# MoZhou1995/DeepPDE_ActorCritic

Measured on AMD Instinct MI355X. Metric: SDE trajectory-steps/sec (batch×horizon) at d=20; value-fn rel-L2 vs analytic, higher is better.
Workload: dtype f32

## Files before the change

### deeppde_actorcritic_amd/csrc/dpac_device.h

```cpp
#pragma once

#include <hip/hip_runtime.h>
#include <rocrand/rocrand_kernel.h>
#include <stdint.h>

#include "dpac.h"
#include "dpac_mfma.h"

namespace dpac {

__host__ __device__ constexpr int pow2_at_least(int v) {
  int p = 1;
  while (p < v) p *= 2;
  return p;
}
#ifndef DPAC_LANE_CAP
#define DPAC_LANE_CAP 16
#endif
#ifndef DPAC_LANE_COMPS
#define DPAC_LANE_COMPS 2
#endif
__host__ __device__ constexpr int lanes_for_dim(int D) {
  return pow2_at_least((D + DPAC_LANE_COMPS - 1) / DPAC_LANE_COMPS) < DPAC_LANE_CAP
             ? pow2_at_least((D + DPAC_LANE_COMPS - 1) / DPAC_LANE_COMPS)
             : DPAC_LANE_CAP;
}
__host__ __device__ constexpr int comps_per_lane(int D) {
  return (D + lanes_for_dim(D) - 1) / lanes_for_dim(D);
}
__host__ __device__ constexpr int eqn_lanes(int eqn, int D) {
  return eqn == DPAC_EQN_VDP ? 1 : lanes_for_dim(D);
}

template <int D, int P>
struct Own {
  static constexpr int M = (D + P - 1) / P;
  static constexpr bool kFull = (D % M) == 0;
  int p;
  __device__ __forceinline__ explicit Own(int p_) : p(p_) {}
  __device__ __forceinline__ int j(int m) const { return p * M + m; }
  __device__ __forceinline__ bool valid(int m) const { return p * M + m < D; }
  __device__ __forceinline__ bool active() const { return p * M < D; }
  template <typename T>
  __device__ __forceinline__ void mask(T (&v)[M]) const {
#pragma unroll
    for (int m = 0; m < M; ++m) v[m] = valid(m) ? v[m] : T(0);
  }
  template <typename T>
  __device__ __forceinline__ void load_masked(const T* __restrict__ row, T (&v)[M]) const {
#pragma unroll
    for (int m = 0; m < M; ++m) v[m] = valid(m) ? row[p * M + m] : T(0);
  }
  template <typename T>
  __device__ __forceinline__ void store(T* __restrict__ row, const T (&v)[M]) const {
#pragma unroll
    for (int m = 0; m < M; ++m)
      if (valid(m)) row[p * M + m] = v[m];
  }
};

struct TdRows {
  const void *x, *u, *dw;
  int64_t ldx;
  int ldu, p;
  double sa, sb;
  void* gdot;
  const void* g_gdot;
};

constexpr uint32_t kOOB = 0x80000000u;
constexpr int kRsrcFlags = 0x00020000;

__device__ __forceinline__ __amdgpu_buffer_rsrc_t make_rsrc(const void* base, uint32_t bytes) {
  return __builtin_amdgcn_make_buffer_rsrc(const_cast<void*>(base), 0, (int)bytes, kRsrcFlags);
}

constexpr float kX3Range = 32768.f;
__device__ __forceinline__ bool x3_bad4(float a, float b, float c, float d) {
  return !(fabsf(a) < kX3Range) | !(fabsf(b) < kX3Range) | !(fabsf(c) < kX3Range) | !(fabsf(d) < kX3Range);
}
__device__ __forceinline__ bool x3_bad(float a) { return !(fabsf(a) < kX3Range); }
__device__ __forceinline__ void x3_flag(uint32_t* st) {
  if (st) __hip_atomic_fetch_or(st, 1u, __ATOMIC_RELAXED, __HIP_MEMORY_SCOPE_AGENT);
}
__device__ __forceinline__ bool x3_status_set(const uint32_t* st) {
  return st && __hip_atomic_load(const_cast<uint32_t*>(st), __ATOMIC_RELAXED, __HIP_MEMORY_SCOPE_AGENT) != 0u;
}
// ... 101 lines not shown
      for (int m = 0; m < M; ++m) {
        uint32_t w[sizeof(T) / 4];
        buf_load_dwords<sizeof(T) / 4, AUX>(r, off[m], w, soff);
        __builtin_memcpy(&v[m], &w[0], sizeof(T));
      }
    }
  }
  template <int AUX = 0>
  __device__ __forceinline__ void store(__amdgpu_buffer_rsrc_t r, const T (&v)[M], uint32_t soff = 0) const {
    if constexpr (kVec) {
      uint32_t w[K];
      __builtin_memcpy(&w[0], &v[0], sizeof(w));
      buf_store_dwords<K, AUX>(r, off[0], w, soff);
    } else {
#pragma unroll
      for (int m = 0; m < M; ++m) {
        uint32_t w[sizeof(T) / 4];
        __builtin_memcpy(&w[0], &v[m], sizeof(T));
        buf_store_dwords<sizeof(T) / 4, AUX>(r, off[m], w, soff);
      }
    }
  }
};

template <int CTRL>
__device__ __forceinline__ int dpp_i32(int v) {
  return __builtin_amdgcn_mov_dpp(v, CTRL, 0xF, 0xF, true);
}
template <int CTRL>
__device__ __forceinline__ float dpp(float v) {
  return __builtin_bit_cast(float, dpp_i32<CTRL>(__builtin_bit_cast(int, v)));
}
template <int CTRL>
__device__ __forceinline__ double dpp(double v) {
  const long long b = __builtin_bit_cast(long long, v);
  const int lo = dpp_i32<CTRL>(static_cast<int>(b));
  const int hi = dpp_i32<CTRL>(static_cast<int>(b >> 32));
  return __builtin_bit_cast(double,
                            (static_cast<long long>(hi) << 32) | static_cast<unsigned int>(lo));
}
enum : int {
  kDppXor1 = 0xB1,
  kDppXor2 = 0x4E,
  kDppHalfMirror = 0x141,
  kDppMirror = 0x140,
};

__device__ __forceinline__ float row_pair_sum(float v) {
  const unsigned u = __builtin_bit_cast(unsigned, v);
  const auto sw = __builtin_amdgcn_permlane16_swap(u, u, false, false);
  return __builtin_bit_cast(float, (unsigned)sw[0]) + __builtin_bit_cast(float, (unsigned)sw[1]);
}
__device__ __forceinline__ double row_pair_sum(double v) {
  const unsigned long long u = __builtin_bit_cast(unsigned long long, v);
  const unsigned lo = (unsigned)u, hi = (unsigned)(u >> 32);
  const auto sl = __builtin_amdgcn_permlane16_swap(lo, lo, false, false);
  const auto sh = __builtin_amdgcn_permlane16_swap(hi, hi, false, false);
  const double a = __builtin_bit_cast(double, ((unsigned long long)(unsigned)sh[0] << 32) | (unsigned)sl[0]);
  const double b = __builtin_bit_cast(double, ((unsigned long long)(unsigned)sh[1] << 32) | (unsigned)sl[1]);
  return a + b;
}

template <int P, typename T>
__device__ __forceinline__ T group_shift_in(T keep, T v, bool group_start) {
  if constexpr (P == 1) {
    return v;
  } else {
    constexpr int kRowShr1 = 0x111;
    T sh;
    if constexpr (sizeof(T) == 4) {
      sh = __builtin_bit_cast(T, __builtin_amdgcn_update_dpp(__builtin_bit_cast(int, v),
                                                            __builtin_bit_cast(int, keep),
                                                            kRowShr1, 0xF, 0xF, false));
    } else {
      const long long vb = __builtin_bit_cast(long long, v), kb = __builtin_bit_cast(long long, keep);
      const int lo = __builtin_amdgcn_update_dpp((int)vb, (int)kb, kRowShr1, 0xF, 0xF, false);
      const int hi = __builtin_amdgcn_update_dpp((int)(vb >> 32), (int)(kb >> 32), kRowShr1, 0xF, 0xF,
                                                 false);
      sh = __builtin_bit_cast(T, ((long long)hi << 32) | (unsigned int)lo);
    }
    if constexpr (P < 16) sh = group_start ? v : sh;
    return sh;
  }
}

template <int P>
struct Lanes {
  static_assert(P == 1 || P == 2 || P == 4 || P == 8 || P == 16 || P == 32, "bad group size");
  template <typename T>
  __device__ __forceinline__ static T sum(T v) {
    if constexpr (P >= 2) v = v + dpp<kDppXor1>(v);
    if constexpr (P >= 4) v = v + dpp<kDppXor2>(v);
    if constexpr (P >= 8) v = v + dpp<kDppHalfMirror>(v);
    if constexpr (P >= 16) v = v + dpp<kDppMirror>(v);
    if constexpr (P >= 32) v = row_pair_sum(v);
    return v;
  }
};

enum : uint64_t { kTagDw = 0, kTagDir = 1, kTagRadius = 2, kTagBdry = 3 };

__device__ __forceinline__ uint4 philox_block(uint64_t seed, uint64_t subseq, uint64_t block) {
  rocrand_state_philox4x32_10 st;
  rocrand_init(seed, subseq, block * 4ull, &st);
  return rocrand4(&st);
}

__device__ __forceinline__ void box_muller_hw(unsigned int x, unsigned int y, float& a, float& b) {
  const float u = ROCRAND_2POW32_INV + (x * ROCRAND_2POW32_INV);
  const float v = ROCRAND_2POW32_INV_2PI + (y * ROCRAND_2POW32_INV_2PI);
  const float s = __builtin_amdgcn_sqrtf(-2.0f * __logf(u));
  float sn, cs;
  __sincosf(v, &sn, &cs);
  a = sn * s;
  b = cs * s;
}

template <typename T>
struct Rng;
template <>
struct Rng<float> {
  static constexpr int kNormalPerBlock = 4;
  __device__ __forceinline__ static void normals(uint4 v, float (&o)[4]) {
    box_muller_hw(v.x, v.y, o[0], o[1]);
    box_muller_hw(v.z, v.w, o[2], o[3]);
  }
};
template <>
struct Rng<double> {
  static constexpr int kNormalPerBlock = 2;
  __device__ __forceinline__ static void normals(uint4 v, double (&o)[2]) {
    const double2 n = rocrand_device::detail::normal_distribution_double2(v);
    o[0] = n.x;
    o[1] = n.y;
  }
};

template <typename T>
__device__ __forceinline__ T bounded_value(unsigned int w) {
  const unsigned int k = static_cast<unsigned int>((static_cast<unsigned long long>(w) * 6ull) >> 32);
  const T s3 = static_cast<T>(1.7320508075688772);
  return k == 0u ? -s3 : (k == 5u ? s3 : static_cast<T>(0));
}

template <typename T>
__host__ __device__ constexpr int dw_per_block(int sample_type) {
  return sample_type == DPAC_SAMPLE_BOUNDED ? 4 : (sizeof(T) == 4 ? 4 : 2);
}

template <typename T>
__host__ __device__ constexpr int dw_steps_per_block(int M, int sample_type) {
  return 2 * M <= dw_per_block<T>(sample_type) ? 2 : 1;
}

template <typename T>
__device__ __forceinline__ void dw_block_values(uint64_t seed, uint64_t traj, uint64_t block,
                                                int sample_type, T (&v)[4]) {
  const uint4 w = philox_block(seed, traj, (kTagDw << 48) | block);
  if (sample_type == DPAC_SAMPLE_BOUNDED) {
    v[0] = bounded_value<T>(w.x); v[1] = bounded_value<T>(w.y);
    v[2] = bounded_value<T>(w.z); v[3] = bounded_value<T>(w.w);
  } else {
    T n[Rng<T>::kNormalPerBlock];
    Rng<T>::normals(w, n);
#pragma unroll
    for (int e = 0; e < Rng<T>::kNormalPerBlock; ++e) v[e] = n[e];
// ... 285 lines not shown
  __device__ __forceinline__ void Lop(const T* v, T* o) const {
#pragma unroll
    for (int i = 0; i < C; ++i) o[i] = two_a * v[i] - eps * (v[nxt(i)] + v[prv(i)]);
  }
  __device__ __forceinline__ void u_true(const T (&x)[M], T, T (&u)[MC]) const {
    T dv2[C];
    Lop(x + C, dv2);
#pragma unroll
    for (int i = 0; i < C; ++i) u[i] = -dv2[i] / 2 / q;
  }
  __device__ __forceinline__ void drift(const T (&x)[M], const T (&u)[MC], T, T (&f)[M]) const {
#pragma unroll
    for (int i = 0; i < C; ++i) {
      const T x1 = x[i], x2 = x[C + i];
      f[i] = x2;
      f[C + i] = (1 - x1 * x1) * x2 - x1 + u[i];
    }
  }
  __device__ __forceinline__ void sigma(const T (&x)[M], const T (&u)[MC], T (&s)[M]) const {
#pragma unroll
    for (int m = 0; m < M; ++m) s[m] = sqrt2;
  }
  static void sigma_form(const dpac_eqn_params&, double& sa, double& sb) { sa = 1.4142135623730951; sb = 0.0; }
  __device__ __forceinline__ T w_part(const T (&x)[M], const T (&u)[MC]) const {
    T dv1[C], dv2[C];
    Lop(x, dv1);
    Lop(x + C, dv2);
    T acc = 0;
#pragma unroll
    for (int i = 0; i < C; ++i) {
      const T x1 = x[i], x2 = x[C + i];
      const T px1 = x[nxt(i)], px2 = x[C + nxt(i)];
      const T temp = geps * (x1 * px1 + x2 * px2) + (dv2[i] * dv2[i]) / 4 / q - x2 * dv1[i] -
                     ((1 - x1 * x1) * x2 - x1) * dv2[i];
      acc += temp + q * (u[i] * u[i]) + ga * (x1 * x1 + x2 * x2);
    }
    return acc;
  }
  __device__ __forceinline__ T w_finish(T s) const { return s - two_ad; }
  __device__ __forceinline__ T V_true(const T (&x)[M], T S, T r) const {
    T cross = 0;
#pragma unroll
    for (int i = 0; i < C; ++i) cross += x[i] * x[nxt(i)] + x[C + i] * x[C + nxt(i)];
    return a * S - eps * cross;
  }
  __device__ __forceinline__ T Z(const T (&x)[M], T S, T r) const { return V_true(x, S, r); }
  __device__ __forceinline__ void V_grad(const T (&x)[M], T S, T r, T (&g)[M]) const {
    Lop(x, g);
    Lop(x + C, g + C);
  }
  __device__ __forceinline__ void drift_vjp(const T (&x)[M], const T (&u)[MC], T r, const T (&a)[M],
                            T (&gx)[M], T (&gu)[MC]) const {
#pragma unroll
    for (int i = 0; i < C; ++i) {
      const T x1 = x[i], x2 = x[C + i], a1 = a[i], a2v = a[C + i];
      gx[i] += a2v * (-2 * x1 * x2 - 1);
      gx[C + i] += a1 + a2v * (1 - x1 * x1);
      gu[i] += a2v;
    }
  }
  __device__ __forceinline__ void sigma_vjp(const T (&x)[M], const T (&u)[MC], const T (&a)[M], T (&gx)[M],
                            T (&gu)[MC]) const {}
  __device__ __forceinline__ void w_vjp(const T (&x)[M], const T (&u)[MC], T gw, T (&gx)[M], T (&gu)[MC]) const {
    T dv1[C], dv2[C], g[C], Ldv2[C], Lg[C];
    Lop(x, dv1);
    Lop(x + C, dv2);
#pragma unroll
    for (int i = 0; i < C; ++i) g[i] = (1 - x[i] * x[i]) * x[C + i] - x[i];
    Lop(dv2, Ldv2);
    Lop(g, Lg);
#pragma unroll
    for (int i = 0; i < C; ++i) {
      const T x1 = x[i], x2 = x[C + i];
      const T s1 = x[nxt(i)] + x[prv(i)], s2 = x[C + nxt(i)] + x[C + prv(i)];
      const T d1 = geps * s1 + 2 * x1 * x2 * dv2[i] + two_ga * x1;
      const T d2 = geps * s2 + Ldv2[i] * inv2q - dv1[i] - (1 - x1 * x1) * dv2[i] - Lg[i] + two_ga * x2;
      gx[i] += gw * d1;
      gx[C + i] += gw * d2;
      gu[i] += gw * (two_q * u[i]);
    }
  }
};

}
```

### deeppde_actorcritic_amd/csrc/dpac_eqn_lqr.hip

```cpp
#include "dpac_kernels.h"

namespace dpac {
template <typename T, int D>
using EqLQRFor = EqLQR<T, D, eqn_lanes(DPAC_EQN_LQR, D)>;
namespace {
const Registrar<EqLQRFor, std::conditional_t<DPAC_TU_DOUBLE, double, float>, DPAC_DIMS> reg(DPAC_EQN_LQR);
}
}

#if DPAC_NN_TRACE && DPAC_TU_TRACE
extern "C" int dpac_debug_trace(void* host, int64_t bytes) {
  const int64_t n = bytes < (int64_t)sizeof(dpac::g_nn_trace) ? bytes : (int64_t)sizeof(dpac::g_nn_trace);
  return (int)hipMemcpyFromSymbol(host, HIP_SYMBOL(dpac::g_nn_trace), (size_t)n, 0, hipMemcpyDeviceToHost);
}
#endif
```

### deeppde_actorcritic_amd/csrc/dpac_kernels.h

```cpp
#pragma once

#include <cmath>
#include <type_traits>
#include <utility>

#include "dpac_device.h"

namespace dpac {

enum Op : int {
  OP_ROLLOUT = 0,
  OP_FLAG_INIT,
  OP_STEP_FWD,
  OP_STEP_BWD,
  OP_TD_FWD,
  OP_TD_BWD,
  OP_EVAL,
  OP_ROLLOUT_NN,
  OP_ROLLOUT_NN_BWD,
};

inline int nn_mask_tile_bytes(int n_hidden) { return 13 * 64 * n_hidden; }

struct OpArgs {
  int op;
  dpac_eqn_params eq;
  int scheme, dtype, td_type, cost_order, sample_type, what;
  int64_t B, traj_offset;
  int N;
  double T;
  uint64_t seed;
  const void *x0, *dw, *x, *u, *dt_in, *coef_in, *G, *disc_in, *y_in;
  const int32_t* flag_in;
  const void *g_x_out, *g_disc_out, *g_y_out;
  void *x_out, *dt, *coef, *u_out, *y, *disc, *disc_out, *y_out;
  int32_t* flag_out;
  void *g_x, *g_u, *g_disc, *g_G, *out;
  dpac_mlp mlp;
  void *save_z, *save_disc;
  int32_t* save_flag;
  uint8_t* save_mask;
  int32_t* mask_written;
  const uint8_t* mask_in;
  const void* mlp_wt[DPAC_MLP_MAX_HIDDEN + 1];
  hipStream_t stream;
};

inline HostConsts host_consts(const OpArgs& a) {
  HostConsts h;
  const double d = a.eq.dim;
  h.gamma = a.eq.gamma;
  h.R = a.eq.R;
  h.sigma_up = a.eq.sigma_up;
  h.dt0 = a.T / a.N;
  h.sqrt_dt0 = std::sqrt(h.dt0);
  h.dt_min = h.dt0 * 1e-4;
  h.den = 3 * a.eq.dim * (a.eq.sigma_up * a.eq.sigma_up);
  h.c_layer = a.eq.sigma_up * std::sqrt(3 * d * h.dt0);
  h.R2 = a.eq.R * a.eq.R;
  return h;
}

template <typename T>
struct DevConsts {
  T gamma, R, dt0, sqrt_dt0, dt_min, inv_den, two_inv_den, c_layer, R2, neg_gamma;
  static DevConsts make(const HostConsts& h) {
    DevConsts c;
    c.gamma = (T)h.gamma; c.R = (T)h.R; c.dt0 = (T)h.dt0; c.sqrt_dt0 = (T)h.sqrt_dt0;
    c.dt_min = (T)h.dt_min; c.inv_den = (T)(1.0 / h.den); c.two_inv_den = (T)(2.0 / h.den);
    c.c_layer = (T)h.c_layer; c.R2 = (T)h.R2; c.neg_gamma = (T)(-h.gamma);
    return c;
  }
};

#ifndef DPAC_RING_VGPRS
#define DPAC_RING_VGPRS 32
#endif
#ifndef DPAC_ROLLOUT_KB_CAP
#define DPAC_ROLLOUT_KB_CAP 8
#endif
#ifndef DPAC_ROLLOUT_DW_AUX
#define DPAC_ROLLOUT_DW_AUX 0
#endif
#ifndef DPAC_ROLLOUT_X_AUX
#define DPAC_ROLLOUT_X_AUX 2
// ... 240 lines not shown
#pragma unroll
            for (int m = 0; m < M; ++m) {
              fr.dw[m] = v[m];
              pend[m] = v[M + m];
            }
          } else {
#pragma unroll
            for (int m = 0; m < M; ++m) fr.dw[m] = pend[m];
          }
          return;
        }
      }
      draw_owned<T, E, D>(a.seed, gtraj, t, lc.p, a.sample_type, fr.dw);
    } else if constexpr (DPAC_ABLATE == 2 || DPAC_ABLATE == 5) {
#pragma unroll
      for (int m = 0; m < M; ++m) fr.dw[m] = T(((t * 7 + m + lc.p) & 3) - 1.5) * T(0.5);
    } else {
      sx.template load<DPAC_ROLLOUT_DW_AUX>(rs_dw, fr.dw, (uint32_t)t * slab);
    }
  };
  auto body = [&](int t, DwFrame<T, M>& fr, auto phase) {
    T dwv[M];
#pragma unroll
    for (int m = 0; m < M; ++m) dwv[m] = fr.dw[m];
    if constexpr (PHILOX) own.mask(dwv);
    T u[MC];
    eq.u_true(x, r, u);
    TR tr;
    tr.run(eq, c, x, u, dwv, fl, r);
    const T cf = tr.coef ? T(1) : T(0);
    if constexpr (COST) {
      const T w = eq.w_finish(Lanes<P>::sum(eq.w_part(x, u)));
      y += cost_increment(a.cost_order, w, cf, tr.dt, disc);
      disc = disc * disc_factor(tr.dt, cf, c);
    }
#pragma unroll
    for (int m = 0; m < M; ++m) x[m] = tr.coef ? tr.xt[m] : x[m];
    if constexpr (TR::kRadius) r = tr.coef ? tr.rt : r;
    fl = tr.next;
    if constexpr (DPAC_ABLATE == 1 || DPAC_ABLATE == 5) {
      if (t + 1 == a.N) sx.store(rs_x, x, (uint32_t)(t + 1) * slab);
      return;
    }
    if constexpr (DPAC_ABLATE != 4) sx.template store<DPAC_ROLLOUT_X_AUX>(rs_x, x, (uint32_t)(t + 1) * slab);
    if constexpr (WANT_U) su.store(rs_u, u, (uint32_t)t * slab_u);
    if constexpr (DPAC_ABLATE != 3) {
      constexpr int PH = decltype(phase)::value;
      keep = group_shift_in<P>(keep, tr.coef ? tr.dt : -tr.dt, lc.p == 0);
      if constexpr (PH >= 0) {
        if constexpr (PH % F == F - 1) flush(t, F);
      } else if ((t & (F - 1)) == F - 1) {
        flush(t, F);
      }
    }
  };
  pipelined<KB, DwFrame<T, M>>(0, a.N, load, body);
  if constexpr (DPAC_ABLATE != 3 && DPAC_ABLATE != 1 && DPAC_ABLATE != 5) {
    const int rem = a.N & (F - 1);
    if (rem) flush(a.N - 1, rem);
  }
  if constexpr (COST) {
    if (lc.live && lc.p == 0) {
      a.y[lc.b] = y;
      a.disc[lc.b] = disc;
    }
  }
}

#ifndef DPAC_ST_CHUNKS
#define DPAC_ST_CHUNKS 4
#endif
#ifndef DPAC_ST_TIGHT
#define DPAC_ST_TIGHT 0
#endif
#ifndef DPAC_ST_TIGHT_CHUNKS
#define DPAC_ST_TIGHT_CHUNKS 3
#endif
#ifndef DPAC_ST_PD
#define DPAC_ST_PD 1
#endif
constexpr int kStCW = 4;
constexpr int kStCH = 16;
constexpr int kStPD = DPAC_ST_PD;
static_assert(kStPD >= 1 && kStPD <= kStCH, "prefetch distance within a chunk");
template <typename T, int D, int P>
struct StagedPlan {
  static constexpr int TPW = kStCW * (64 / P);
  static constexpr int SLOT = TPW * D * (int)sizeof(T);
  static constexpr int PIECES = (SLOT + 1023) / 1024;
  static constexpr int kLdsCap = 128 * 1024;
  static constexpr int SLOT_1K = (SLOT + 16 + 1023) / 1024 * 1024;
  static constexpr int SLOT_16 = (SLOT + 16 + 15) / 16 * 16;
  static constexpr bool kWide = !DPAC_ST_TIGHT && DPAC_ST_CHUNKS * kStCH * SLOT_1K <= kLdsCap;
  static constexpr int CHUNKS = kWide ? DPAC_ST_CHUNKS : DPAC_ST_TIGHT_CHUNKS;
  static constexpr int SLOT_LDS = kWide ? SLOT_1K : SLOT_16;
  static constexpr int PADOFF = SLOT_LDS - 16;
  static constexpr int RS = CHUNKS * kStCH;
  static_assert(P < 4 || (SLOT % 16 == 0 && (PIECES - 1) * 1024 + 16 <= SLOT), "DMA pieces stay inside the slot");
  static constexpr bool kOk = P >= 4 && RS * SLOT_LDS <= kLdsCap && kStCH * PIECES <= 62;
};

template <class Fn, int... S>
__device__ __forceinline__ void unroll_phases(Fn& fn, std::integer_sequence<int, S...>) {
  (fn(Phase<S>{}), ...);
}

__device__ __forceinline__ int lds_load_relaxed(const int* p) {
  return __hip_atomic_load(p, __ATOMIC_RELAXED, __HIP_MEMORY_SCOPE_WORKGROUP);
}
__device__ __forceinline__ void lds_store_relaxed(int* p, int v) {
  __hip_atomic_store(p, v, __ATOMIC_RELAXED, __HIP_MEMORY_SCOPE_WORKGROUP);
}

template <int GEN>
constexpr int st_waves() { return kStCW + (GEN > 0 ? GEN : 1); }
#ifndef DPAC_ST_GEN
#define DPAC_ST_GEN 12
#endif
constexpr int kStGen = DPAC_ST_GEN;

template <typename T, class E, int D, int SCHEME, int OUT, int KB, int GEN = 0>
__global__ __launch_bounds__(64 * st_waves<GEN>()) void k_rollout_staged(const E eq, const DevConsts<T> c,
                                                                          const RolloutArgs<T> a) {
  constexpr int P = E::kP, M = E::M, MC = E::MC;
  using PL = StagedPlan<T, D, P>;
  constexpr int TPW = PL::TPW, RS = PL::RS, PIECES = PL::PIECES, SLOT_LDS = PL::SLOT_LDS;
  constexpr bool COST = (OUT & kOutCost) != 0, WANT_U = (OUT & kOutU) != 0;
  constexpr int F = P < kStCH ? P : kStCH;
  constexpr int NREADY = GEN > 0 ? GEN : 1;
  static_assert(kStCH % F == 0 && (F & (F - 1)) == 0, "flush phase fixed per unrolled body");
  static_assert(GEN == 0 || (2 * M <= 4 && kStCH % 2 == 0), "generators draw the paired layout");
  using TR = Transition<T, E, SCHEME>;
  __shared__ __attribute__((aligned(16))) unsigned char s_ring[RS * SLOT_LDS];
  __shared__ int s_ready[NREADY], s_done[kStCW];
  const int wave = __builtin_amdgcn_readfirstlane((int)threadIdx.x / 64), lane = (int)threadIdx.x % 64;
  const int64_t row0 = xcd_block(blockIdx.x, gridDim.x) * TPW;
  const int N = a.N;
  if (threadIdx.x == 0) {
#pragma unroll
    for (int w = 0; w < NREADY; ++w) s_ready[w] = 0;
#pragma unroll
    for (int w = 0; w < kStCW; ++w) s_done[w] = 0;
  }
  if (threadIdx.x < RS * 4)
    reinterpret_cast<uint32_t*>(s_ring + (threadIdx.x / 4) * SLOT_LDS + PL::PADOFF)[threadIdx.x % 4] = 0u;
  __syncthreads();

  if constexpr (GEN > 0) {
    if (wave >= kStCW) {
      const int g = wave - kStCW;
      const int64_t rows_live = (a.B - row0) < TPW ? (a.B - row0) : TPW;
      constexpr int PLS = (D + M - 1) / M;
      constexpr int NBLK = (kStCH / 2) * TPW * PLS;
      constexpr int PASSES = (NBLK + 64 * GEN - 1) / (64 * GEN);
      constexpr int SLOT_T = SLOT_LDS / (int)sizeof(T);
      T* const ringw = reinterpret_cast<T*>(s_ring);
      for (int c0 = 0; c0 < N; c0 += kStCH) {
        const int need = c0 + kStCH - RS;
        if (need > 0) {
          for (;;) {
            int mn = lds_load_relaxed(&s_done[0]);
#pragma unroll
            for (int w = 1; w < kStCW; ++w) mn = min(mn, lds_load_relaxed(&s_done[w]));
            if (mn >= need) break;
            __builtin_amdgcn_s_sleep(2);
          }
        }
        asm volatile("" ::: "memory");
#pragma unroll 1
        for (int k = 0; k < PASSES; ++k) {
          const int e = (k * GEN + g) * 64 + lane;
          const int u = e / (TPW * PLS), rem = e - u * (TPW * PLS);
          const int i = rem / PLS, p = rem - i * PLS;
          const int t0 = c0 + 2 * u;
          if (e < NBLK && t0 < N && i < rows_live) {
            T v[4];
            dw_block_values<T>(a.seed, (uint64_t)(a.traj_offset + row0 + i), (uint64_t)(t0 >> 1) * P + p,
                               a.sample_type, v);
            T* d0 = ringw + (t0 % RS) * SLOT_T + i * D + p * M;
            T* d1 = ringw + ((t0 + 1) % RS) * SLOT_T + i * D + p * M;
#pragma unroll
            for (int m = 0; m < M; ++m) {
              if (p * M + m < D) {
                d0[m] = v[m];
                if (t0 + 1 < N) d1[m] = v[M + m];
              }
            }
          }
        }
        asm volatile("s_waitcnt lgkmcnt(0)" ::: "memory");
        if (lane == 0) lds_store_relaxed(&s_ready[g], c0 + kStCH < N ? c0 + kStCH : N);
      }
      return;
    }
  } else if (wave == kStCW) {
    const int64_t rows_live = (a.B - row0) < TPW ? (a.B - row0) : TPW;
    const uint32_t bytes = (uint32_t)(rows_live * D * (int64_t)sizeof(T));
    const uint32_t lds0 = (uint32_t)(uintptr_t)(__attribute__((address_space(3))) unsigned char*)s_ring;
    const char* base = (const char*)(a.dw + row0 * D);
    const int64_t step_bytes = a.B * D * (int64_t)sizeof(T);
    for (int c0 = 0; c0 < N; c0 += kStCH) {
      const int need = c0 + kStCH - RS;
      if (need > 0) {
        for (;;) {
          int mn = lds_load_relaxed(&s_done[0]);
#pragma unroll
          for (int w = 1; w < kStCW; ++w) mn = min(mn, lds_load_relaxed(&s_done[w]));
          if (mn >= need) break;
          __builtin_amdgcn_s_sleep(2);
        }
      }
      asm volatile("" ::: "memory");
#pragma unroll
      for (int s = 0; s < kStCH; ++s) {
        const int t = c0 + s < N ? c0 + s : N - 1;
        const char* src = base + t * step_bytes;
        const uint32_t slot = lds0 + (uint32_t)((t % RS) * SLOT_LDS);
#pragma unroll
        for (int k = 0; k < PIECES; ++k) {
          const uint32_t off = (uint32_t)((k * 64 + lane) * 16);
          const char* gp = src + (off < bytes ? off : 0u);
          const uint32_t m0 = __builtin_amdgcn_readfirstlane(slot + (uint32_t)(k * 1024));
          if (off < bytes || lane == 0) {
            int keep;
            asm volatile("s_mov_b32 %0, m0\n\ts_mov_b32 m0, %2\n\ts_nop 0\n\tglobal_load_lds_dwordx4 %1, off\n\ts_mov_b32 m0, %0"
                         : "=&s"(keep) : "v"(gp), "s"(m0) : "memory");
          }
        }
      }
      if (c0 > 0) {
        asm volatile("s_waitcnt vmcnt(%0)" ::"n"(kStCH * PIECES) : "memory");
        if (lane == 0) lds_store_relaxed(&s_ready[0], c0);
      }
    }
    asm volatile("s_waitcnt vmcnt(0)" ::: "memory");
    if (lane == 0) lds_store_relaxed(&s_ready[0], N);
    return;
  }

  const LaneCoord<P> lc(a.B, lane, row0 + wave * (64 / P));
  const int gl = wave * (64 / P) + lane / P;
  const Own<D, P> own(lc.p);
  const Own<E::CDIM, P> ownu(lc.p);
  const BufSlab<T, D, P> sx(own, lc.b, lc.live);
  const BufSlab<T, E::CDIM, P> su(ownu, lc.b, lc.live);
  const uint32_t slab = (uint32_t)(a.B * D * sizeof(T));
  const uint32_t slab_u = (uint32_t)(a.B * E::CDIM * sizeof(T));
  const uint32_t row_bytes = (uint32_t)(N * sizeof(T));
  const __amdgpu_buffer_rsrc_t rs_x = make_rsrc(a.x, slab * (uint32_t)(N + 1));
  const __amdgpu_buffer_rsrc_t rs_u = make_rsrc(a.u, WANT_U ? slab_u * (uint32_t)N : 0u);
  const __amdgpu_buffer_rsrc_t rs_dt = make_rsrc(a.dt, (uint32_t)a.B * row_bytes);
  const __amdgpu_buffer_rsrc_t rs_cf = make_rsrc(a.coef, (uint32_t)a.B * row_bytes);
  const T* ring = reinterpret_cast<const T*>(s_ring);
  const int lds_e = gl * D + lc.p * M;
  constexpr bool kVecRead = Own<D, P>::kFull && (M * sizeof(T) == 8 || M * sizeof(T) == 16);
  const uint32_t lane_off = own.active() ? (uint32_t)(lds_e * (int)sizeof(T)) : (uint32_t)PL::PADOFF;
  T keep = 0;
  auto flush = [&](int t_last, int count) {
    const uint32_t off = (lc.live && lc.p < count)
                             ? (uint32_t)((lc.b * N + t_last - lc.p) * (int64_t)sizeof(T)) : kOOB;
    buf_store_scalar<T>(rs_dt, off, fabs(keep));
    buf_store_scalar<T>(rs_cf, off, keep > T(0) ? T(1) : T(0));
  };
  T x[M];
  sx.load(make_rsrc(a.x0, slab), x);
  sx.store(rs_x, x);
  T r = TR::kRadius ? dsqrt(Lanes<P>::sum(sumsq(x))) : T(0);
  Flags fl = SCHEME == DPAC_SCHEME_ADAPTIVE ? region(r, c) : Flags{true, false};
  T disc = 1, y = 0;
  auto read_dw_at = [&](int t, uint32_t slot_bytes, T (&dwv)[M]) {
    if constexpr (kVecRead) {
      typedef T vec __attribute__((ext_vector_type(M)));
      const vec v = *reinterpret_cast<const vec*>(s_ring + slot_bytes + lane_off);
#pragma unroll
      for (int m = 0; m < M; ++m) dwv[m] = v[m];
    } else {
      const T* slot = ring + (t % RS) * (SLOT_LDS / (int)sizeof(T)) + lds_e;
#pragma unroll
      for (int m = 0; m < M; ++m) dwv[m] = own.valid(m) ? slot[m] : T(0);
    }
  };
  auto read_dw = [&](int t, T (&dwv)[M]) { read_dw_at(t, (uint32_t)((t % RS) * SLOT_LDS), dwv); };
  auto body = [&](int t, const T (&dwv)[M], auto phase) {
    T u[MC];
    eq.u_true(x, r, u);
    TR tr;
    tr.run(eq, c, x, u, dwv, fl, r);
    const T cf = tr.coef ? T(1) : T(0);
    if constexpr (COST) {
      const T w = eq.w_finish(Lanes<P>::sum(eq.w_part(x, u)));
      y += cost_increment(a.cost_order, w, cf, tr.dt, disc);
      disc = disc * disc_factor(tr.dt, cf, c);
    }
#pragma unroll
    for (int m = 0; m < M; ++m) x[m] = tr.coef ? tr.xt[m] : x[m];
    if constexpr (TR::kRadius) r = tr.coef ? tr.rt : r;
    fl = tr.next;
    sx.template store<DPAC_ROLLOUT_X_AUX>(rs_x, x, (uint32_t)(t + 1) * slab);
    if constexpr (WANT_U) su.store(rs_u, u, (uint32_t)t * slab_u);
    constexpr int PH = decltype(phase)::value;
    keep = group_shift_in<P>(keep, tr.coef ? tr.dt : -tr.dt, lc.p == 0);
    if constexpr (PH >= 0) {
      if constexpr (PH % F == F - 1) flush(t, F);
    } else if ((t & (F - 1)) == F - 1) {
      flush(t, F);
    }
  };
  for (int c0 = 0; c0 < N; c0 += kStCH) {
    const int want = c0 + kStCH < N ? c0 + kStCH : N;
    for (;;) {
      int mn = lds_load_relaxed(&s_ready[0]);
#pragma unroll
      for (int w = 1; w < NREADY; ++w) mn = min(mn, lds_load_relaxed(&s_ready[w]));
      if (mn >= want) break;
      __builtin_amdgcn_s_sleep(1);
    }
    asm volatile("" ::: "memory");
    if (c0 + kStCH <= N) {
      const uint32_t cb = (uint32_t)__builtin_amdgcn_readfirstlane((c0 % RS) * SLOT_LDS);
      constexpr int PD = kStPD;
      T nxt[PD][M];
#pragma unroll
      for (int q = 0; q < PD; ++q) read_dw_at(c0 + q, cb + (uint32_t)(q * SLOT_LDS), nxt[q]);
      auto one = [&](auto sidx) {
        constexpr int S = decltype(sidx)::value;
        T cur[M];
#pragma unroll
        for (int m = 0; m < M; ++m) cur[m] = nxt[S % PD][m];
        if constexpr (S + PD < kStCH) read_dw_at(c0 + S + PD, cb + (uint32_t)((S + PD) * SLOT_LDS), nxt[S % PD]);
        if constexpr (PD > 1) __builtin_amdgcn_sched_barrier(0);
        body(c0 + S, cur, Phase<S>{});
      };
      unroll_phases(one, std::make_integer_sequence<int, kStCH>{});
    } else {
      for (int t = c0; t < N; ++t) {
        T cur[M];
        read_dw(t, cur);
        body(t, cur, Phase<-1>{});
      }
    }
    asm volatile("s_waitcnt lgkmcnt(0)" ::: "memory");
    if (lane == 0) lds_store_relaxed(&s_done[wave], want);
  }
  const int rem = N & (F - 1);
  if (rem) flush(N - 1, rem);
  if constexpr (COST) {
    if (lc.live && lc.p == 0) {
      a.y[lc.b] = y;
      a.disc[lc.b] = disc;
    }
  }
}

template <typename T, class E, int D, int SCHEME>
__global__ __launch_bounds__(64) void k_flag_init(const E eq, const DevConsts<T> c, int64_t B,
                                                   const T* x0, int32_t* flag) {
  constexpr int P = E::kP, M = E::M;
  const LaneCoord<P> lc(B, threadIdx.x, xcd_block(blockIdx.x, gridDim.x) * (64 / P));
  const Own<D, P> own(lc.p);
  T xv[M];
  own.load_masked(x0 + lc.b * D, xv);
  const T r = dsqrt(Lanes<P>::sum(sumsq(xv)));
  if (lc.p == 0) flag[lc.b] = SCHEME == DPAC_SCHEME_ADAPTIVE ? region(r, c).encode() : 1;
}

template <typename T>
struct StepArgs {
  int64_t B;
  int cost_order;
  const T *x, *u, *dw, *disc_in, *y_in;
  const int32_t* flag_in;
  T *x_out, *disc_out, *y_out, *dt, *coef;
  int32_t* flag_out;
  const T *g_x_out, *g_disc_out, *g_y_out;
  T *g_x, *g_u, *g_disc;
};

template <typename T, class E, int D, int SCHEME>
__global__ __launch_bounds__(64) void k_step_fwd(const E eq, const DevConsts<T> c,
                                                  const StepArgs<T> a) {
  constexpr int P = E::kP, M = E::M, MC = E::MC;
  using TR = Transition<T, E, SCHEME>;
  const LaneCoord<P> lc(a.B, threadIdx.x, xcd_block(blockIdx.x, gridDim.x) * (64 / P));
  const Own<D, P> own(lc.p);
  const Own<E::CDIM, P> ownu(lc.p);
  T x[M], u[MC], dw[M];
  own.load_masked(a.x + lc.b * D, x);
  own.load_masked(a.dw + lc.b * D, dw);
  ownu.load_masked(a.u + lc.b * E::CDIM, u);
  const T r = TR::kRadius ? dsqrt(Lanes<P>::sum(sumsq(x))) : T(0);
  const Flags fl = Flags::decode(a.flag_in[lc.b]);
  const T disc = a.disc_in ? a.disc_in[lc.b] : T(1);
  TR tr;
  tr.run(eq, c, x, u, dw, fl, r);
  const T cf = tr.coef ? T(1) : T(0);
  const T w = eq.w_finish(Lanes<P>::sum(eq.w_part(x, u)));
  T xn[M];
#pragma unroll
  for (int m = 0; m < M; ++m) xn[m] = tr.coef ? tr.xt[m] : x[m];
  own.store(a.x_out + lc.b * D, xn);
  if (lc.p == 0) {
    const T yin = a.y_in ? a.y_in[lc.b] : T(0);
    if (a.y_out) a.y_out[lc.b] = yin + cost_increment(a.cost_order, w, cf, tr.dt, disc);
    if (a.disc_out) a.disc_out[lc.b] = disc * disc_factor(tr.dt, cf, c);
    if (a.dt) a.dt[lc.b] = tr.dt;
    if (a.coef) a.coef[lc.b] = cf;
    a.flag_out[lc.b] = SCHEME == DPAC_SCHEME_ADAPTIVE ? tr.next.encode() : (tr.coef ? 1 : 0);
  }
}

template <typename T, class E, int SCHEME>
__device__ __forceinline__ void step_vjp(const E& eq, const DevConsts<T>& c, const T (&x)[E::M],
                                         const T (&u)[E::MC], const T (&dw)[E::M], Flags fl,
                                         T disc, const T (&lam)[E::M], T gD1, T gy1,
                                         T (&gx)[E::M], T (&gu)[E::MC], T& g_disc) {
  constexpr int P = E::kP, M = E::M, MC = E::MC;
  using TR = Transition<T, E, SCHEME>;
  const T r = dsqrt(Lanes<P>::sum(sumsq(x)));
  TR tr;
  tr.run(eq, c, x, u, dw, fl, r);
  const T cf = tr.coef ? T(1) : T(0);
  const T w = eq.w_finish(Lanes<P>::sum(eq.w_part(x, u)));
  const T Ef = disc_factor(tr.dt, cf, c);

  T f[M], s[M];
  eq.drift(x, u, r, f);
  eq.sigma(x, u, s);
  T a_f[M], a_s[M];
// ... 666 lines not shown
```

Baseline: 27.30 billion.

## Add specialized inline step with carried dt and radius state in staged rollout

Replaces the generic Transition-based step in the staged rollout with a hand-written step lambda. It keeps a running candidate state, a running radius bound, and a precomputed next dt and sqrt(dt), so each step avoids recomputing the region and adaptive step size from scratch. It also adds optional tracing instrumentation (disabled by default) and a pin helper and ConstSigma trait, neither of which is used yet. The new path is on by default via DPAC_ST_STEP; the rewritten exit and layer logic risks diverging numerically from the original Transition.

```diff
diff --git a/deeppde_actorcritic_amd/csrc/dpac_device.h b/deeppde_actorcritic_amd/csrc/dpac_device.h
--- a/deeppde_actorcritic_amd/csrc/dpac_device.h
+++ b/deeppde_actorcritic_amd/csrc/dpac_device.h
@@ -3,6 +3,8 @@
 #include <hip/hip_runtime.h>
 #include <rocrand/rocrand_kernel.h>
 #include <stdint.h>
+
+#include <type_traits>
 
 #include "dpac.h"
 #include "dpac_mfma.h"
@@ -270,6 +272,16 @@
     if constexpr (P < 16) sh = group_start ? v : sh;
     return sh;
   }
+}
+
+template <typename T>
+__device__ __forceinline__ void pin(T& v) {
+  asm volatile("" : "+v"(v));
+}
+template <typename T, typename... Ts>
+__device__ __forceinline__ void pin(T& v, Ts&... more) {
+  pin(v);
+  pin(more...);
 }
 
 template <int P>
@@ -721,4 +733,11 @@
   }
 };
 
-}
+template <class E>
+struct ConstSigma : std::false_type {};
+template <typename T, int D, int P>
+struct ConstSigma<EqLQR<T, D, P>> : std::true_type {};
+template <typename T, int D, int P>
+struct ConstSigma<EqEKN<T, D, P>> : std::true_type {};
+
+}
diff --git a/deeppde_actorcritic_amd/csrc/dpac_eqn_lqr.hip b/deeppde_actorcritic_amd/csrc/dpac_eqn_lqr.hip
--- a/deeppde_actorcritic_amd/csrc/dpac_eqn_lqr.hip
+++ b/deeppde_actorcritic_amd/csrc/dpac_eqn_lqr.hip
@@ -14,3 +14,10 @@
   return (int)hipMemcpyFromSymbol(host, HIP_SYMBOL(dpac::g_nn_trace), (size_t)n, 0, hipMemcpyDeviceToHost);
 }
 #endif
+
+#if DPAC_ST_TRACE && DPAC_TU_TRACE
+extern "C" int dpac_debug_staged_trace(void* host, int64_t bytes) {
+  const int64_t n = bytes < (int64_t)sizeof(dpac::g_st_trace) ? bytes : (int64_t)sizeof(dpac::g_st_trace);
+  return (int)hipMemcpyFromSymbol(host, HIP_SYMBOL(dpac::g_st_trace), (size_t)n, 0, hipMemcpyDeviceToHost);
+}
+#endif
diff --git a/deeppde_actorcritic_amd/csrc/dpac_kernels.h b/deeppde_actorcritic_amd/csrc/dpac_kernels.h
--- a/deeppde_actorcritic_amd/csrc/dpac_kernels.h
+++ b/deeppde_actorcritic_amd/csrc/dpac_kernels.h
@@ -1,6 +1,7 @@
 #pragma once
 
 #include <cmath>
+#include <limits>
 #include <type_traits>
 #include <utility>
 
@@ -407,6 +408,10 @@
 constexpr int kStCW = 4;
 constexpr int kStCH = 16;
 constexpr int kStPD = DPAC_ST_PD;
+#ifndef DPAC_ST_STEP
+#define DPAC_ST_STEP 1
+#endif
+constexpr bool kOwnStep = DPAC_ST_STEP != 0;
 static_assert(kStPD >= 1 && kStPD <= kStCH, "prefetch distance within a chunk");
 template <typename T, int D, int P>
 struct StagedPlan {
@@ -444,6 +449,42 @@
 #endif
 constexpr int kStGen = DPAC_ST_GEN;
 
+#ifndef DPAC_ST_TRACE
+#define DPAC_ST_TRACE 0
+#endif
+#if DPAC_ST_TRACE
+constexpr int kStTraceRow = 128, kStTraceWaves = 16, kStTraceChunks = 32;
+static __device__ uint32_t g_st_trace[2 * kStTraceWaves * kStTraceRow];
+__device__ __forceinline__ uint32_t st_clock() {
+  unsigned long long t;
+  __builtin_amdgcn_sched_barrier(0);
+  asm volatile("s_memtime %0\n\ts_waitcnt lgkmcnt(0)" : "=s"(t)::"memory");
+  __builtin_amdgcn_sched_barrier(0);
+  return (uint32_t)t;
+}
+__device__ __forceinline__ uint32_t st_realtime() {
+  unsigned long long t;
+  __builtin_amdgcn_sched_barrier(0);
+  asm volatile("s_memrealtime %0\n\ts_waitcnt lgkmcnt(0)" : "=s"(t)::"memory");
+  __builtin_amdgcn_sched_barrier(0);
+  return (uint32_t)t;
+}
+#define ST_PUT(pt, v)                \
+  do {                               \
+    const uint32_t st_v_ = (v);      \
+    if (st_on) st_row[(pt)] = st_v_; \
+  } while (0)
+#define ST_MARK(pt) ST_PUT(pt, st_clock())
+#define ST_CHUNK(base, c0) ((base) + ((c0) / kStCH < kStTraceChunks ? (c0) / kStCH : kStTraceChunks - 1))
+#else
+#define ST_PUT(pt, v) \
+  do {                \
+  } while (0)
+#define ST_MARK(pt) \
+  do {              \
+  } while (0)
+#endif
+
 template <typename T, class E, int D, int SCHEME, int OUT, int KB, int GEN = 0>
 __global__ __launch_bounds__(64 * st_waves<GEN>()) void k_rollout_staged(const E eq, const DevConsts<T> c,
                                                                           const RolloutArgs<T> a) {
@@ -461,6 +502,12 @@
   const int wave = __builtin_amdgcn_readfirstlane((int)threadIdx.x / 64), lane = (int)threadIdx.x % 64;
   const int64_t row0 = xcd_block(blockIdx.x, gridDim.x) * TPW;
   const int N = a.N;
+#if DPAC_ST_TRACE
+  const bool st_on = lane == 0 && wave < kStTraceWaves && (blockIdx.x == 0 || blockIdx.x == gridDim.x - 1);
+  uint32_t* const st_row = g_st_trace + ((blockIdx.x == 0 ? 0 : kStTraceWaves) + (wave < kStTraceWaves ? wave : 0)) * kStTraceRow;
+  ST_MARK(0);
+  ST_PUT(5, st_realtime());
+#endif
   if (threadIdx.x == 0) {
 #pragma unroll
     for (int w = 0; w < NREADY; ++w) s_ready[w] = 0;
@@ -470,6 +517,7 @@
   if (threadIdx.x < RS * 4)
     reinterpret_cast<uint32_t*>(s_ring + (threadIdx.x / 4) * SLOT_LDS + PL::PADOFF)[threadIdx.x % 4] = 0u;
   __syncthreads();
+  ST_MARK(1);
 
   if constexpr (GEN > 0) {
     if (wave >= kStCW) {
@@ -536,6 +584,9 @@
         }
       }
       asm volatile("" ::: "memory");
+#if DPAC_ST_TRACE
+      ST_MARK(ST_CHUNK(16, c0));
+#endif
 #pragma unroll
       for (int s = 0; s < kStCH; ++s) {
         const int t = c0 + s < N ? c0 + s : N - 1;
@@ -553,13 +604,21 @@
           }
         }
       }
+#if DPAC_ST_TRACE
+      ST_MARK(ST_CHUNK(48, c0));
+#endif
       if (c0 > 0) {
         asm volatile("s_waitcnt vmcnt(%0)" ::"n"(kStCH * PIECES) : "memory");
         if (lane == 0) lds_store_relaxed(&s_ready[0], c0);
+#if DPAC_ST_TRACE
+        ST_MARK(ST_CHUNK(80, c0));
+#endif
       }
     }
     asm volatile("s_waitcnt vmcnt(0)" ::: "memory");
     if (lane == 0) lds_store_relaxed(&s_ready[0], N);
+    ST_MARK(4);
+    ST_PUT(6, st_realtime());
     return;
   }
 
@@ -593,6 +652,19 @@
   T r = TR::kRadius ? dsqrt(Lanes<P>::sum(sumsq(x))) : T(0);
   Flags fl = SCHEME == DPAC_SCHEME_ADAPTIVE ? region(r, c) : Flags{true, false};
   T disc = 1, y = 0;
+  T xc[M], rc = r;
+#pragma unroll
+  for (int m = 0; m < M; ++m) xc[m] = x[m];
+  T Ra = fl.alive ? c.R : -std::numeric_limits<T>::infinity();
+  bool alive = fl.alive;
+  const T sq0 = SCHEME == DPAC_SCHEME_ADAPTIVE ? dsqrt(c.dt0) : c.sqrt_dt0;
+  T dt = c.dt0, sq = sq0;
+  if constexpr (kOwnStep && SCHEME == DPAC_SCHEME_ADAPTIVE) {
+    dt = adaptive_dt_raw(fl.layer, r, c);
+    dt = fl.layer ? fmax(dt, c.dt_min) : dt;
+    sq = dsqrt(dt);
+  }
+  ST_MARK(2);
   auto read_dw_at = [&](int t, uint32_t slot_bytes, T (&dwv)[M]) {
     if constexpr (kVecRead) {
       typedef T vec __attribute__((ext_vector_type(M)));
@@ -631,8 +703,67 @@
       flush(t, F);
     }
   };
+  auto step = [&](int t, const T (&dwv)[M], auto phase) {
+    T uc[MC], f[M], s[M], xt[M];
+    eq.u_true(xc, rc, uc);
+    eq.drift(xc, uc, rc, f);
+    eq.sigma(xc, uc, s);
+#pragma unroll
+    for (int m = 0; m < M; ++m) xt[m] = xc[m] + fma(f[m], dt, (s[m] * dwv[m]) * sq);
+    const T St = Lanes<P>::sum(sumsq(xt));
+    T u[MC];
+    if constexpr (COST || WANT_U) eq.u_true(x, r, u);
+    bool coef;
+    T rt = T(0), dtn = dt, sqn = sq;
+    if constexpr (SCHEME == DPAC_SCHEME_ADAPTIVE) {
+      rt = dsqrt(St);
+      const T b = Ra - rt;
+      const bool inner = b - c.c_layer > T(0);
+      coef = b > T(0);
+      const T dtb = fmax((b * b) * c.inv_den, c.dt_min);
+      const T sqb = dsqrt(dtb);
+      const bool layer = coef && !inner;
+      dtn = layer ? dtb : c.dt0;
+      sqn = layer ? sqb : sq0;
+      Ra = coef ? Ra : -std::numeric_limits<T>::infinity();
+    } else {
+      if constexpr (E::kNeedsNorm) rt = dsqrt(St);
+      coef = alive && !(St - c.R2 >= T(0));
+      alive = coef;
+    }
+    if constexpr (COST) {
+      const T cf = coef ? T(1) : T(0);
+      const T w = eq.w_finish(Lanes<P>::sum(eq.w_part(x, u)));
+      y += cost_increment(a.cost_order, w, cf, dt, disc);
+      disc = disc * disc_factor(dt, cf, c);
+    }
+    const T kv = coef ? dt : -dt;
+#pragma unroll
+    for (int m = 0; m < M; ++m) {
+      x[m] = coef ? xt[m] : x[m];
+      xc[m] = xt[m];
+    }
+    if constexpr (E::kNeedsNorm) {
+      r = coef ? rt : r;
+      rc = rt;
+    }
+    dt = dtn;
+    sq = sqn;
+    sx.template store<DPAC_ROLLOUT_X_AUX>(rs_x, x, (uint32_t)(t + 1) * slab);
+    if constexpr (WANT_U) su.store(rs_u, u, (uint32_t)t * slab_u);
+    constexpr int PH = decltype(phase)::value;
+    keep = group_shift_in<P>(keep, kv, lc.p == 0);
+    if constexpr (PH >= 0) {
+      if constexpr (PH % F == F - 1) flush(t, F);
+    } else if ((t & (F - 1)) == F - 1) {
+      flush(t, F);
+    }
+  };
   for (int c0 = 0; c0 < N; c0 += kStCH) {
     const int want = c0 + kStCH < N ? c0 + kStCH : N;
+#if DPAC_ST_TRACE
+    const uint32_t st_poll0 = st_clock();
+#endif
     for (;;) {
       int mn = lds_load_relaxed(&s_ready[0]);
 #pragma unroll
@@ -641,6 +772,14 @@
       __builtin_amdgcn_s_sleep(1);
     }
     asm volatile("" ::: "memory");
+#if DPAC_ST_TRACE
+    {
+      const uint32_t st_now = st_clock();
+      ST_PUT(ST_CHUNK(16, c0), st_now);
+      ST_PUT(ST_CHUNK(80, c0), st_now - st_poll0);
+      if (c0 == 0) ST_PUT(3, st_now);
+    }
+#endif
     if (c0 + kStCH <= N) {
       const uint32_t cb = (uint32_t)__builtin_amdgcn_readfirstlane((c0 % RS) * SLOT_LDS);
       constexpr int PD = kStPD;
@@ -654,21 +793,36 @@
         for (int m = 0; m < M; ++m) cur[m] = nxt[S % PD][m];
         if constexpr (S + PD < kStCH) read_dw_at(c0 + S + PD, cb + (uint32_t)((S + PD) * SLOT_LDS), nxt[S % PD]);
         if constexpr (PD > 1) __builtin_amdgcn_sched_barrier(0);
-        body(c0 + S, cur, Phase<S>{});
+        if constexpr (kOwnStep)
+          step(c0 + S, cur, Phase<S>{});
+        else
+          body(c0 + S, cur, Phase<S>{});
       };
       unroll_phases(one, std::make_integer_sequence<int, kStCH>{});
     } else {
       for (int t = c0; t < N; ++t) {
         T cur[M];
         read_dw(t, cur);
-        body(t, cur, Phase<-1>{});
+        if constexpr (kOwnStep)
+          step(t, cur, Phase<-1>{});
+        else
+          body(t, cur, Phase<-1>{});
       }
     }
     asm volatile("s_waitcnt lgkmcnt(0)" ::: "memory");
     if (lane == 0) lds_store_relaxed(&s_done[wave], want);
+#if DPAC_ST_TRACE
+    ST_MARK(ST_CHUNK(48, c0));
+#endif
   }
   const int rem = N & (F - 1);
   if (rem) flush(N - 1, rem);
+#if DPAC_ST_TRACE
+  ST_MARK(4);
+  asm volatile("s_waitcnt vmcnt(0)" ::: "memory");
+  ST_MARK(7);
+  ST_PUT(6, st_realtime());
+#endif
   if constexpr (COST) {
     if (lc.live && lc.p == 0) {
       a.y[lc.b] = y;
```

Result: faster. 27.67 billion, median of 6 (+1.4%).
